# XiaokunSun/SemanticHuman

Measured on AMD Instinct MI355X. Metric: training meshes/sec at 6890 verts, batch=64, higher is better.
Workload: dtype f32

## Files before the change

include/sh_kernels.h:

```cpp
#ifndef SH_KERNELS_H
#define SH_KERNELS_H

#include <stddef.h>
#include <stdint.h>

#ifdef __cplusplus
extern "C" {
#endif

typedef void* sh_stream_t;

#if defined(__GNUC__)
#define SH_API __attribute__((visibility("default")))
#else
#define SH_API
#endif

enum sh_status {
    SH_OK = 0,
    SH_ERR_INVALID_ARG = -1,
    SH_ERR_UNSUPPORTED = -2,
    SH_ERR_WORKSPACE = -3,
    SH_ERR_LAUNCH = -4
};
// ... 142 lines not shown
SH_API int sh_grouped_linear_bwd_wgt(int G, const float* dy, int64_t y_rs, const int64_t* y_off, const float* x,
                              int64_t x_rs, const int64_t* x_off, float* const* dW, float* const* dbias, int M,
                              const int* N, const int* K, sh_stream_t stream);

SH_API size_t sh_reduce_workspace(void);

SH_API int sh_l1_loss_fwd(const float* a, const float* b, int64_t n, float* loss, void* workspace, sh_stream_t stream);
SH_API int sh_l1_loss_bwd(const float* a, const float* b, int64_t n, const float* gscale, float* grad_b, sh_stream_t stream);

SH_API int sh_vertex_l2(const float* a, const float* b, int B, int N1, int N, float scale, float* out,
                 void* workspace, sh_stream_t stream);

SH_API int sh_edge_ratio_loss_fwd(const float* x_hat, const float* x, const int32_t* faces, int B, int N1, int F,
                           float* loss, void* workspace, sh_stream_t stream);
SH_API int sh_edge_ratio_loss_bwd(const float* x_hat, const float* x, const int32_t* faces,
                           const int32_t* vptr, const int32_t* vcorner, int B, int N1, int F,
                           const float* gscale, float* grad, sh_stream_t stream);

SH_API size_t sh_recon_loss_workspace(void);
SH_API int sh_recon_loss_fwd(const float* x_hat, const float* x, const int32_t* faces, int B, int N1, int F, float edge_w,
                      float* total, float* parts, void* workspace, sh_stream_t stream);
SH_API int sh_recon_loss_bwd(const float* x_hat, const float* x, const int32_t* vptr, const int32_t* vnbr, int B, int N1, int F,
                      float edge_w, const float* gscale, float* grad, sh_stream_t stream);

SH_API int sh_part_pairdist_tile_rows(void);
SH_API int sh_part_pairdist_loss_fwd(const float* x_rec, const float* x_gt, const float* bone, const float* scale,
                              const int32_t* part_ptr, const int32_t* part_vert, const int32_t* tile_ptr,
                              const int32_t* flags, const float* w_part, int B, int N1, int P, int T, int max_part,
                              int w_mode, float w_threshold, int relat, float* loss, float* part_sum, float* part_cnt,
                              void* workspace, size_t workspace_bytes, sh_stream_t stream);
SH_API int sh_part_pairdist_loss_bwd(const float* x_rec, const float* x_gt, const float* bone, const float* scale,
                              const int32_t* part_ptr, const int32_t* part_vert, const int32_t* tile_ptr,
                              const int32_t* flags, const float* w_part, int B, int N1, int P, int T, int max_part,
                              int w_mode, float w_threshold, int relat, const float* part_cnt, const float* gscale,
                              float* grad, sh_stream_t stream);
SH_API int sh_part_pairdist_loss_fwd_grad(const float* x_rec, const float* x_gt, const float* bone, const float* scale,
                                   const int32_t* part_ptr, const int32_t* part_vert, const int32_t* tile_ptr, const int32_t* flags,
                                   const float* w_part, int B, int N1, int P, int T, int max_part, int w_mode, float w_threshold,
                                   int relat, float* loss, float* part_sum, float* part_cnt, float* grad_raw, void* workspace,
                                   size_t workspace_bytes, sh_stream_t stream);
SH_API int sh_part_pairdist_loss_bwd_scale(const float* grad_raw, const int32_t* part_ptr, const int32_t* part_vert,
                                   const float* w_part, const float* part_cnt, const float* gscale, int B, int N1, int P,
                                   int n_part_verts, float* grad, sh_stream_t stream);

SH_API int sh_measure_girth(const float* v, int64_t v_sb, const int32_t* ring_ptr, const int32_t* ring_a,
                     const int32_t* ring_b, const float* ring_f, int B, int P, float* girth, sh_stream_t stream);
// ... 186 lines not shown
SH_API int sh_spiral_conv_p3_grp(const void* xp, const int32_t* g_rows, const uint32_t* g_pos, const int32_t* g_out, int n_groups, int g_L,
                                 const void* wfrag3, const float* bias, float* y, int64_t y_sv, int64_t y_sb, void* yp, const float* yprev,
                                 int64_t yp_sv, int64_t yp_sb, const void* yprev_planes, int act, int zero_row, int backward, int B, int R,
                                 int S, int Cg, int Nout, sh_stream_t stream);

SH_API int sh_spiral_conv_bf16_rag_ok(int B, int S, int Cg, int Nout, int rag_L);
SH_API int sh_spiral_conv_bwd_data_bf16_rag(const void* dpre, int64_t dp_sv, int64_t dp_sb, const int32_t* rag_rows, const int32_t* rag_pos,
                                            int rag_L, const void* wfrag_t, void* dx, int64_t dx_sv, int64_t dx_sb, const void* yprev,
                                            int64_t yp_sv, int64_t yp_sb, int act_prev, int zero_row, int B, int n_in, int S, int Cin,
                                            int Cout, sh_stream_t stream);

SH_API int sh_spiral_conv_bwd_wgt_p3_ok(int B, int R, int S, int Cin, int Cout);
SH_API size_t sh_spiral_conv_bwd_wgt_p3_workspace(int B, int R, int S, int Cin, int Cout);
SH_API int sh_spiral_conv_bwd_wgt_p3(const void* dpre_planes, int dpre_zero_row, const void* x_planes, const int32_t* table, void* workspace,
                                     size_t workspace_bytes, int B, int R, int S, int Cin, int Cout, sh_stream_t stream);
SH_API int sh_spiral_conv_bwd_wgt_p3_presum(const void* dpre_planes, int dpre_zero_row, const void* x_planes, const int32_t* table,
                                            void* workspace, size_t workspace_bytes, const float* dpre, int64_t dp_sv, int64_t dp_sb,
                                            const int32_t* sum_rowptr, const int32_t* sum_col, const float* sum_val, float* sum_out,
                                            void* sum_out_planes, int sum_rows, int B, int R, int S, int Cin, int Cout,
                                            sh_stream_t stream);
SH_API int sh_spiral_conv_bwd_wgt_reduce_multi_kinds(int n_layers, const void* const* workspaces, float* const* dW, float* const* dbias,
                                                     const int* B, const int* R, const int* S, const int* Cin, const int* Cout,
                                                     const int* kinds, sh_stream_t stream);

#ifdef __cplusplus
}
#endif
#endif
```

semantichuman_amd/_lib.py:

```python
from __future__ import annotations

import ctypes
import os
from ctypes import c_char_p, c_float, c_int, c_int64, c_size_t, c_void_p

_HERE = os.path.dirname(os.path.abspath(__file__))
LIB_PATH = os.environ.get("SH_KERNEL_LIB") or os.path.join(_HERE, "lib", "libsh_kernels.so")

ACT_IDS = {"identity": 0, "relu": 1, "elu": 2, "leaky_relu": 3, "sigmoid": 4, "tanh": 5}

_P, _I, _L = c_void_p, c_int, c_int64
SIGNATURES = {
    "sh_version": (c_int, []),
    "sh_last_error": (c_char_p, []),
    "sh_build_id": (c_char_p, []),
    "sh_clock_probe": (c_int, [_P, _I, _I, _P]),
    "sh_profile_enable": (c_int, [_I]),
    "sh_profile_count": (c_int, []),
    "sh_profile_get": (c_int, [_I, c_char_p, _I, ctypes.POINTER(c_float)]),
    "sh_spiral_conv_fwd": (c_int, [_P, _L, _L, _P, _P, _P, _P, _L, _L, _I, _I, _I, _I, _I, _I, _I, _I, _P]),
    "sh_spiral_conv_bwd_data": (c_int, [_P, _L, _L, _P, _P, _P, _L, _L, _P, _L, _L, _I, _I, _I, _I, _I, _I, _I, _I, _P]),
    "sh_spiral_conv_bwd_data_z": (c_int, [_P, _L, _L, _I, _P, _P, _P, _L, _L, _P, _L, _L, _I, _I, _I, _I, _I, _I, _I, _I, _P]),
    "sh_weight_transpose": (c_int, [_P, _P, _I, _I, _I, _P]),
    "sh_spiral_conv_bwd_wgt_workspace": (c_size_t, [_I, _I, _I, _I, _I]),
# ... 8 lines not shown
    "sh_stack_forward": (c_int, [_I, _P, _P, _I, _I, _I, _I, _P, _P, _P, _I, _I, _P, _P, _I, _P]),
    "sh_stack_backward": (c_int, [_I, _P, _P, _I, _I, _I, _I, _P, _P, _I, _P, _P, _P, _P, _P, _P, _P, _P, _I, _I, _P, _P, _P, _P, _I, _P]),
    "sh_linear_workspace": (c_size_t, [_I, _I, _I]),
    "sh_linear_fwd": (c_int, [_P, _P, _P, _P, _I, _I, _I, _P, c_size_t, _I, _P]),
    "sh_linear_bwd_data": (c_int, [_P, _P, _P, _I, _I, _I, _P, c_size_t, _I, _P]),
    "sh_linear_bwd_wgt": (c_int, [_P, _P, _P, _P, _I, _I, _I, _P, c_size_t, _I, _P]),
    "sh_linear_bwd_wgt_adam_ok": (c_int, [_I, _I, _I]),
    "sh_linear_bwd_wgt_adam": (c_int, [_P, _I, _P, _I] + [_P] * 6 + [ctypes.c_double] * 4 + [_P, _I, _I, _I, _I, _P]),
    "sh_adam_bump": (c_int, [_I, _P, _P]),
    "sh_grouped_linear_fwd": (c_int, [_I, _P, _L, _P, _P, _P, _P, _L, _P, _I, _P, _P, _P]),
    "sh_grouped_linear_bwd_data": (c_int, [_I, _P, _L, _P, _P, _P, _L, _P, _I, _P, _P, _P]),
    "sh_grouped_linear_bwd_wgt": (c_int, [_I, _P, _L, _P, _P, _L, _P, _P, _P, _I, _P, _P, _P]),
    "sh_reduce_workspace": (c_size_t, []),
    "sh_l1_loss_fwd": (c_int, [_P, _P, _L, _P, _P, _P]),
    "sh_l1_loss_bwd": (c_int, [_P, _P, _L, _P, _P, _P]),
    "sh_vertex_l2": (c_int, [_P, _P, _I, _I, _I, c_float, _P, _P, _P]),
    "sh_edge_ratio_loss_fwd": (c_int, [_P, _P, _P, _I, _I, _I, _P, _P, _P]),
    "sh_edge_ratio_loss_bwd": (c_int, [_P, _P, _P, _P, _P, _I, _I, _I, _P, _P, _P]),
    "sh_spiral_conv_bwd_wgt_thin_ok": (c_int, [_I, _I, _I, _I, _I, _I]),
    "sh_spiral_conv_bwd_wgt_thin": (c_int, [_P, _L, _L, _P, _I, _L, _L, _P, _P, c_size_t, _P, _P, _L, _L, _P, _I, _I, _I, _I, _I, _I, _I, _I, _I, _P]),
    "sh_recon_loss_workspace": (c_size_t, []),
    "sh_recon_loss_fwd": (c_int, [_P, _P, _P, _I, _I, _I, c_float, _P, _P, _P, _P]),
    "sh_recon_loss_bwd": (c_int, [_P, _P, _P, _P, _I, _I, _I, c_float, _P, _P, _P]),
    "sh_part_pairdist_tile_rows": (c_int, []),
    "sh_part_pairdist_loss_fwd": (c_int, [_P] * 9 + [_I] * 6 + [c_float, _I, _P, _P, _P, _P, c_size_t, _P]),
    "sh_part_pairdist_loss_bwd": (c_int, [_P] * 9 + [_I] * 6 + [c_float, _I, _P, _P, _P, _P]),
    "sh_part_pairdist_loss_fwd_grad": (c_int, [_P] * 9 + [_I] * 6 + [c_float, _I, _P, _P, _P, _P, _P, c_size_t, _P]),
    "sh_part_pairdist_loss_bwd_scale": (c_int, [_P] * 6 + [_I] * 4 + [_P, _P]),
    "sh_measure_girth": (c_int, [_P, _L, _P, _P, _P, _P, _I, _I, _P, _P]),
    "sh_bone_length": (c_int, [_P, _P, _I, _I, _I, _P, _P]),
    "sh_measure_girth_bwd": (c_int, [_P, _L, _P, _P, _P, _P, _P, _P, _P, _P, _I, _P, _I, _I, _I, _P, _P]),
    "sh_bone_length_bwd": (c_int, [_P, _P, _P, _P, _P, _I, _P, _I, _I, _I, _P, _P]),
    "sh_joint_regress_bwd": (c_int, [_P, _P, _I, _I, _I, _I, _P, _P]),
    "sh_nearest_points_chunks": (c_int, [_I, _I, _I]),
    "sh_nearest_points_workspace": (c_size_t, [_I, _I, _I, _I]),
    "sh_nearest_points": (c_int, [_P, _L, _I, _P, _P, _L, _I, _P, _P, _L, _I, _I, _P, _P, _P, c_size_t, _P]),
    "sh_chamfer_fwd": (c_int, [_P, _I, _P, _P, _I, _I, _P, _L, c_float, c_float, _I, _P, _P, _P]),
    "sh_chamfer_bwd": (c_int, [_P, _L, _I, _I, _P, _L, _I, _P, _P, _P, _P, _P, _P, _L, _P, c_float, c_float, _P, _I, _P, _P]),
    "sh_nearest_surface_chunks": (c_int, [_I, _I, _I]),
    "sh_nearest_surface_workspace": (c_size_t, [_I, _I, _I, _I]),
    "sh_nearest_surface": (c_int, [_P, _L, _I, _P, _P, _L, _I, _P, _I, _P, _L, _P, _I, _I, _I, _P, _P, _P, _P, _P, c_size_t, _P]),
    "sh_chamfer_surface_bwd": (c_int, [_P, _L, _I, _I, _P, _L, _I, _P, _P, _I, _P, _P, _P, _P, _P, _P, _L, _P, c_float, c_float, _P, _I, _P, _P]),
    "sh_vertex_normals": (c_int, [_P, _L, _I, _P, _I, _P, _P, _I, _P, _P]),
    "sh_nearest_points_gated": (c_int, [_P, _L, _I, _P, _P, _L, _P, _L, _I, _P, _P, _L, _P, _L, c_float, _I, _I, _P, _P, _P, c_size_t, _P]),
    "sh_align_ranges": (c_int, [_I, _I, c_float]),
    "sh_align_partials_bytes": (c_size_t, [_I, _I, _I, c_float]),
# ... 34 lines not shown
    "sh_conv_wfrag3_bytes": (c_size_t, [_I, _I, _I]),
    "sh_conv_wfrag3_prep_multi": (c_int, [_I, _P, _P, _P, _P, _P, _P, _P]),
    "sh_spiral_conv_p3_ok": (c_int, [_I, _I, _I, _I]),
    "sh_spiral_conv_p3_kind": (c_int, [_I, _I, _I, _I]),
    "sh_p3_launch_count": (c_int64, []),
    "sh_spiral_conv_fwd_img": (c_int, [_P, _L, _L, _P, _P, _P, _P, _L, _L, _P, _I, _I, _I, _I, _I, _I, _I, _I, _P]),
    "sh_act_backward_tr_img": (c_int, [_P, _L, _L, _P, _L, _L, _P, _L, _L, _P, _I, _I, _I, _I, _I, _I, _P, _P, _P, _P, _P, _P]),
    "sh_spmm_p3": (c_int, [_P, _P, _P, _P, _L, _L, _P, _L, _L, _P, _P, _L, _L, _I, _I, _I, _I, _I, _P]),
    "sh_spiral_conv_fwd_p3": (c_int, [_P, _P, _P, _P, _P, _L, _L, _P, _I, _I, _I, _I, _I, _I, _I, _P]),
    "sh_spiral_conv_bwd_data_p3": (c_int, [_P, _I, _P, _L, _L, _I, _P, _P, _P, _L, _L, _P, _P, _L, _L, _P, _I, _I, _I, _I, _I, _I, _I, _P]),
    "sh_spiral_conv_p3_rag_ok": (c_int, [_I, _I, _I, _I, _I]),
    "sh_spiral_conv_bf16_rag_ok": (c_int, [_I, _I, _I, _I, _I]),
    "sh_spiral_conv_p3_grp_ok": (c_int, [_I, _I, _I, _I, _I]),
    "sh_spiral_conv_p3_grp_members": (c_int, [_I, _I, _I, _I]),
    "sh_spiral_conv_p3_grp_pays": (c_int, [_I, _I]),
    "sh_spiral_conv_p3_grp": (c_int, [_P, _P, _P, _P, _I, _I, _P, _P, _P, _L, _L, _P, _P, _L, _L, _P, _I, _I, _I, _I, _I, _I, _I, _I, _P]),
    "sh_spiral_conv_bwd_data_bf16_rag": (c_int, [_P, _L, _L, _P, _P, _I, _P, _P, _L, _L, _P, _L, _L, _I, _I, _I, _I, _I, _I, _I, _P]),
    "sh_spiral_conv_bwd_data_p3_rag": (c_int, [_P, _P, _P, _I, _P, _P, _L, _L, _P, _P, _L, _L, _P, _I, _I, _I, _I, _I, _I, _I, _P]),
    "sh_spiral_conv_bwd_wgt_p3_ok": (c_int, [_I, _I, _I, _I, _I]),
    "sh_spiral_conv_bwd_wgt_p3_workspace": (c_size_t, [_I, _I, _I, _I, _I]),
    "sh_spiral_conv_bwd_wgt_p3": (c_int, [_P, _I, _P, _P, _P, c_size_t, _I, _I, _I, _I, _I, _P]),
    "sh_spiral_conv_bwd_wgt_p3_presum": (c_int, [_P, _I, _P, _P, _P, c_size_t, _P, _L, _L, _P, _P, _P, _P, _P, _I, _I, _I, _I, _I, _I, _P]),
    "sh_spiral_conv_bwd_wgt_reduce_multi_kinds": (c_int, [_I, _P, _P, _P, _P, _P, _P, _P, _P, _P, _P]),
}
DTYPE_IDS = {"float32": 0, "bfloat16": 1}
FORM = {name: 1 << k for k, name in enumerate(["fwd_p3", "fwd_grp", "fwd_img", "fwd_img_only", "bwd_gimg", "bwd_thin", "bwd_p3", "bwd_rag",
                                                "bwd_grp", "bwd_ride", "bwd_presum_img", "bwd_p3w", "bwd_yimg", "bwd_in_img_only",
                                                "bwd_grad_img_only"])}



class CsrRef(ctypes.Structure):
    _fields_ = [("rowptr", c_void_p), ("col", c_void_p), ("val", c_void_p)]


class StackStep(ctypes.Structure):
    _fields_ = [("kind", c_int), ("param", c_int), ("table", c_void_p), ("table_t", c_void_p),
                ("R", c_int), ("S", c_int), ("n_in", c_int), ("cin", c_int), ("cout", c_int), ("act", c_int), ("zero_row", c_int),
                ("n1", c_int), ("n2", c_int), ("sum1", CsrRef), ("sum2", CsrRef), ("m", CsrRef), ("mt", CsrRef),
                ("m_rows", c_int), ("m_cols", c_int), ("extend", c_int),
                ("rag_rows", c_void_p), ("rag_pos", c_void_p), ("rag_L", c_int),
                ("fg_rows", c_void_p), ("fg_pos", c_void_p), ("fg_out", c_void_p), ("fg_n", c_int), ("fg_L", c_int),
                ("bg_rows", c_void_p), ("bg_pos", c_void_p), ("bg_out", c_void_p), ("bg_n", c_int), ("bg_L", c_int)]


_lib = None
# ... 100 lines not shown
```

semantichuman_amd/csrc/spiral_conv.hip:

```cpp
#include "sh_bf16.h"

#include <type_traits>

int sh_wgrad_bf16_nsplit(int B, int R, int S, int Cin, int Cout);
int sh_wgrad_p3_nslab(int B, int R, int S, int Cin, int Cout);

namespace {

constexpr int TM = 128;
constexpr int KC = 32;
constexpr int NTHREADS = 256;

struct GGParams {
    const float* x; long x_sv, x_sb;
    const int* table;
    const float* w;
    const float* bias;
    float* y; long y_sv, y_sb;
    const float* yprev; long yp_sv, yp_sb;
    int B, R, S, Cg, Nout, K;
    int Kw;
    int act;
    int zero_row;
    int log2TB, n_btiles, n_vtiles, nchunks;
// ... 1107 lines not shown
        for (; r + 48 < nslab; r += 64) {
            const float a = slab[(long)r * stride + i], b = slab[(long)(r + 16) * stride + i];
            const float c = slab[(long)(r + 32) * stride + i], d = slab[(long)(r + 48) * stride + i];
            s += (a + b) + (c + d);
        }
        for (; r < nslab; r += 16) s += slab[(long)r * stride + i];
    }
    red[ry][ox] = s;
    __syncthreads();
    if (ry == 0 && i < n) {
        float t = 0.f;
#pragma unroll
        for (int k = 0; k < 16; ++k) t += red[k][ox];
        out[i] = t;
    }
}

constexpr int MR_MAX = 32;
struct MultiReduce {
    const float* slab[MR_MAX]; long stride[MR_MAX]; long n[MR_MAX]; float* out[MR_MAX];
    int nslab[MR_MAX]; int block0[MR_MAX]; int nd;
    unsigned vec_mask;
};
__global__ __launch_bounds__(1024) void slab_reduce_multi_kernel(const MultiReduce m) {
    __shared__ f32x4 red[16][64];
    int d = 0;
    while (d + 1 < m.nd && m.block0[d + 1] <= (int)blockIdx.x) ++d;
    const float* __restrict__ slab = m.slab[d];
    const long stride = m.stride[d], n = m.n[d];
    const int nslab = m.nslab[d];
    const int ox = threadIdx.x & 63, ry = threadIdx.x >> 6;
    if ((m.vec_mask >> d) & 1u) {
        const long i = ((long)(blockIdx.x - m.block0[d]) * 64 + ox) * 4;
        f32x4 s = {0.f, 0.f, 0.f, 0.f};
        if (i < n) {
            int r = ry;
            for (; r + 48 < nslab; r += 64) {
                const f32x4 a = *reinterpret_cast<const f32x4*>(slab + (long)r * stride + i), b = *reinterpret_cast<const f32x4*>(slab + (long)(r + 16) * stride + i);
                const f32x4 c = *reinterpret_cast<const f32x4*>(slab + (long)(r + 32) * stride + i), e = *reinterpret_cast<const f32x4*>(slab + (long)(r + 48) * stride + i);
                s += (a + b) + (c + e);
            }
            for (; r < nslab; r += 16) s += *reinterpret_cast<const f32x4*>(slab + (long)r * stride + i);
        }
        red[ry][ox] = s;
        __syncthreads();
        if (ry == 0 && i < n) {
            f32x4 t = {0.f, 0.f, 0.f, 0.f};
// ... 3 lines not shown
        }
        return;
    }
    const long i = (long)(blockIdx.x - m.block0[d]) * 64 + ox;
    float s = 0.f;
    if (i < n) {
        int r = ry;
        for (; r + 48 < nslab; r += 64) {
            const float a = slab[(long)r * stride + i], b = slab[(long)(r + 16) * stride + i];
            const float c = slab[(long)(r + 32) * stride + i], e = slab[(long)(r + 48) * stride + i];
            s += (a + b) + (c + e);
        }
        for (; r < nslab; r += 16) s += slab[(long)r * stride + i];
    }
    red[ry][ox][0] = s;
    __syncthreads();
    if (ry == 0 && i < n) {
        float t = 0.f;
#pragma unroll
        for (int k = 0; k < 16; ++k) t += red[k][ox][0];
        m.out[d][i] = t;
    }
}

struct MultiTranspose {
    const float* w[MR_MAX]; float* wt[MR_MAX]; int S[MR_MAX]; int Cin[MR_MAX]; int Cout[MR_MAX]; int block0[MR_MAX]; int nd;
};
__device__ __forceinline__ void weight_transpose_block(const MultiTranspose& m, int blk) {
    int d = 0;
    while (d + 1 < m.nd && m.block0[d + 1] <= blk) ++d;
    const int S = m.S[d], Cin = m.Cin[d], Cout = m.Cout[d];
    const long n = (long)S * Cin * Cout;
    const long i = (long)(blk - m.block0[d]) * 256 + threadIdx.x;
    if (i >= n) return;
    const int co = (int)(i % Cout);
    const long t = i / Cout;
    const int s = (int)(t % S);
    const int ci = (int)(t / S);
    m.wt[d][i] = m.w[d][(long)co * S * Cin + (long)s * Cin + ci];
}
__global__ __launch_bounds__(256) void weight_transpose_multi_kernel(const MultiTranspose m) { weight_transpose_block(m, (int)blockIdx.x); }

struct WSParams {
    const float* dpre; long dp_sv, dp_sb;
    const float* x; long x_sv, x_sb;
    const int* table;
// ... 781 lines not shown
                   "sh_spiral_conv_bwd_wgt: more than 128 output channels (%d) need input channels that are a multiple of 4 (or 3)", Cout);
#define SH_WG_CASE(C, T) rc = launch_wg<C, T>(p, w, vec4, st)
    if (w.ctw == 1) {
        if (w.cot == 1) SH_WG_CASE(1, 1); else if (w.cot == 2) SH_WG_CASE(2, 1); else if (w.cot == 4) SH_WG_CASE(4, 1); else SH_WG_CASE(8, 1);
    } else {
        if (w.cot == 1) SH_WG_CASE(1, 2); else if (w.cot == 2) SH_WG_CASE(2, 2); else if (w.cot == 4) SH_WG_CASE(4, 2); else SH_WG_CASE(8, 2);
    }
    }
#undef SH_WG_CASE
    if (rc != SH_OK) return rc;
    if (!dW) return SH_OK;
    const long n = p.slab_stride;
    ShProfScope ps(st, "slab_reduce_kernel");
    SH_LAUNCH_PS(ps, slab_reduce_kernel, dim3((unsigned)((n + 63) / 64)), dim3(1024), 0, st, p.slab, p.slab_stride, w.nrc, n, dW);
    if (dbias)
        hipLaunchKernelGGL(slab_reduce_kernel, dim3((unsigned)((Cout + 63) / 64)), dim3(1024), 0, st, p.slab + p.bias_off,
                           (long)Cout, w.nrc, (long)Cout, dbias);
    SH_CHECK_LAUNCH("slab_reduce");
    return SH_OK;
}

static int reduce_multi_impl(int n_layers, const void* const* workspaces, float* const* dW, float* const* dbias, const int* B,
                             const int* R, const int* S, const int* Cin, const int* Cout, bool bf16_plan_all, sh_stream_t stream,
                             const int* kinds = nullptr) {
    SH_REQUIRE(n_layers > 0 && 2 * n_layers <= MR_MAX && workspaces && dW && dbias && B && R && S && Cin && Cout,
               SH_ERR_INVALID_ARG, "sh_spiral_conv_bwd_wgt_reduce_multi: bad argument (at most %d layers)", MR_MAX / 2);
    MultiReduce m{};
    int nd = 0, blocks = 0;
    for (int i = 0; i < n_layers; ++i) {
        SH_REQUIRE(workspaces[i] && dW[i], SH_ERR_INVALID_ARG, "sh_spiral_conv_bwd_wgt_reduce_multi: null pointer in layer %d", i);
        const int kind = kinds ? kinds[i] : (bf16_plan_all ? 1 : 0);
        SH_REQUIRE(kind >= 0 && kind <= 2, SH_ERR_INVALID_ARG, "sh_spiral_conv_bwd_wgt_reduce_multi: unknown plan kind %d of layer %d", kind, i);
        const bool bf16_plan = kind == 1;
        const int nrc = kind == 1 ? sh_wgrad_bf16_nsplit(B[i], R[i], S[i], Cin[i], Cout[i])
                        : kind == 2 ? sh_wgrad_p3_nslab(B[i], R[i], S[i], Cin[i], Cout[i]) : plan_wgrad(B[i], R[i], S[i], Cin[i], Cout[i]).nrc;
        SH_REQUIRE(nrc > 0, SH_ERR_UNSUPPORTED, "sh_spiral_conv_bwd_wgt_reduce_multi: layer %d has no plan of kind %d", i, kind);
        const long stride = (long)Cout[i] * S[i] * Cin[i];
        const float* slab = static_cast<const float*>(workspaces[i]);
        m.slab[nd] = slab; m.stride[nd] = stride; m.nslab[nd] = nrc; m.n[nd] = stride; m.out[nd] = dW[i]; m.block0[nd] = blocks;
        static const int vec_on = sh_env_int("SH_SLAB_REDUCE_VEC", 1, 0, 2);
        if ((vec_on == 2 || (vec_on == 1 && (nrc >= 512 || bf16_plan))) && stride % 4 == 0 && ((reinterpret_cast<uintptr_t>(slab) | reinterpret_cast<uintptr_t>(dW[i])) & 15) == 0) {
            m.vec_mask |= 1u << nd;
            blocks += (int)((stride / 4 + 63) / 64);
        } else
            blocks += (int)((stride + 63) / 64);
        ++nd;
        if (dbias[i]) {
            m.slab[nd] = slab + (long)nrc * stride; m.stride[nd] = Cout[i]; m.nslab[nd] = nrc; m.n[nd] = Cout[i];
            m.out[nd] = dbias[i]; m.block0[nd] = blocks;
            blocks += (Cout[i] + 63) / 64; ++nd;
        }
    }
    m.nd = nd;
    hipStream_t st = static_cast<hipStream_t>(stream);
    ShProfScope ps(st, "slab_reduce_multi_kernel");
    SH_LAUNCH_PS(ps, slab_reduce_multi_kernel, dim3((unsigned)blocks), dim3(1024), 0, st, m);
    SH_CHECK_LAUNCH("slab_reduce_multi");
    return SH_OK;
}

int sh_spiral_conv_bwd_wgt_reduce_multi(int n_layers, const void* const* workspaces, float* const* dW, float* const* dbias,
                                        const int* B, const int* R, const int* S, const int* Cin, const int* Cout,
                                        sh_stream_t stream) {
    return reduce_multi_impl(n_layers, workspaces, dW, dbias, B, R, S, Cin, Cout, false, stream);
}

int sh_spiral_conv_bwd_wgt_reduce_multi_kinds(int n_layers, const void* const* workspaces, float* const* dW, float* const* dbias,
                                              const int* B, const int* R, const int* S, const int* Cin, const int* Cout,
                                              const int* kinds, sh_stream_t stream) {
    SH_REQUIRE(kinds, SH_ERR_INVALID_ARG, "sh_spiral_conv_bwd_wgt_reduce_multi_kinds: no kinds");
    return reduce_multi_impl(n_layers, workspaces, dW, dbias, B, R, S, Cin, Cout, false, stream, kinds);
}

int sh_spiral_conv_bwd_wgt_reduce_multi_bf16(int n_layers, const void* const* workspaces, float* const* dW, float* const* dbias,
                                             const int* B, const int* R, const int* S, const int* Cin, const int* Cout,
                                             sh_stream_t stream) {
    return reduce_multi_impl(n_layers, workspaces, dW, dbias, B, R, S, Cin, Cout, true, stream);
}

int sh_weight_transpose_multi(int n_layers, const float* const* weight, float* const* weight_t, const int* S, const int* Cin,
                              const int* Cout, sh_stream_t stream) {
    SH_REQUIRE(n_layers > 0 && n_layers <= MR_MAX && weight && weight_t && S && Cin && Cout, SH_ERR_INVALID_ARG,
               "sh_weight_transpose_multi: bad argument (at most %d layers)", MR_MAX);
    MultiTranspose m{};
    int blocks = 0;
    for (int i = 0; i < n_layers; ++i) {
        SH_REQUIRE(weight[i] && weight_t[i] && S[i] > 0 && Cin[i] > 0 && Cout[i] > 0, SH_ERR_INVALID_ARG,
                   "sh_weight_transpose_multi: bad layer %d", i);
        m.w[i] = weight[i]; m.wt[i] = weight_t[i]; m.S[i] = S[i]; m.Cin[i] = Cin[i]; m.Cout[i] = Cout[i]; m.block0[i] = blocks;
        blocks += (int)(((long)S[i] * Cin[i] * Cout[i] + 255) / 256);
    }
    m.nd = n_layers;
    hipLaunchKernelGGL(weight_transpose_multi_kernel, dim3((unsigned)blocks), dim3(256), 0, static_cast<hipStream_t>(stream), m);
    SH_CHECK_LAUNCH("weight_transpose_multi");
// ... 65 lines not shown
```

semantichuman_amd/csrc/spmm_loss.hip:

```cpp
#include "sh_bf16.h"

namespace {

constexpr int RED_BLOCKS = 2048;

template <bool VEC, bool P3 = false>
__global__ __launch_bounds__(256) void spmm_kernel(const int* __restrict__ rowptr, const int* __restrict__ col,
                                                   const float* __restrict__ val, const float* __restrict__ x, long x_sv, long x_sb,
                                                   float* __restrict__ y, long y_sv, long y_sb, const float* __restrict__ yprev,
                                                   long yp_sv, long yp_sb, int act, int zero_row, int B, int rows, int C,
                                                   char* __restrict__ img = nullptr, long img_vb = 0, long img_bgb = 0) {
    const int CW = VEC ? C >> 2 : C;
    const int per_row = B * CW;
    const int parts = (per_row + 255) >> 8;
    const long items = (long)rows * parts;
    for (long it = blockIdx.x; it < items; it += gridDim.x) {
        const int r = (int)(it / parts), part = (int)(it - (long)r * parts);
        const int e0 = rowptr[r], e1 = rowptr[r + 1];
        const bool zero = r == zero_row;
        for (int j = part * 256 + threadIdx.x; j < per_row && j < (part + 1) * 256; j += 256) {
            const int b = j / CW, cw = j - b * CW;
            const int co = VEC ? 4 * cw : cw;
            const long xo = (long)b * x_sb + co;
            const long yo = (long)r * y_sv + (long)b * y_sb + co;
// ... 219 lines not shown
}

__global__ void edge_loss_bwd_kernel(const float* __restrict__ xh, const float* __restrict__ x, const int* __restrict__ faces,
                                     const int* __restrict__ vptr, const int* __restrict__ vcorner, int B, int N1, int F,
                                     const float* __restrict__ gscale, float* __restrict__ grad) {
    const float sc = gscale[0] / ((float)B * (float)F);
    const long n = (long)B * N1;
    for (long i = (long)blockIdx.x * blockDim.x + threadIdx.x; i < n; i += (long)gridDim.x * blockDim.x) {
        const long bb = i / N1;
        const int v = (int)(i - bb * N1);
        const float* ph = xh + bb * N1 * 3;
        const float* pg = x + bb * N1 * 3;
        float g[3] = {0.f, 0.f, 0.f};
        for (int e = vptr[v]; e < vptr[v + 1]; ++e) {
            const int c = vcorner[e], f = c / 3, kx = c - 3 * f;
            const int o1 = faces[3 * f + (kx + 1) % 3], o2 = faces[3 * f + (kx + 2) % 3];
            edge_grad(ph, pg, v, o1, g);
            edge_grad(ph, pg, v, o2, g);
        }
        grad[i * 3] = sc * g[0]; grad[i * 3 + 1] = sc * g[1]; grad[i * 3 + 2] = sc * g[2];
    }
}

__global__ void recon_partial_kernel(const float* __restrict__ xh, const float* __restrict__ x, const int* __restrict__ faces,
                                     int B, int N1, int F, float* __restrict__ part) {
    __shared__ float red[16];
    float s = 0.f;
    const long n = (long)B * N1 * 3;
    for (long i = (long)blockIdx.x * blockDim.x + threadIdx.x; i < n; i += (long)gridDim.x * blockDim.x) s += fabsf(x[i] - xh[i]);
    const float t1 = block_sum(s, red);
    if (threadIdx.x == 0) part[blockIdx.x] = t1;
    __syncthreads();
    s = 0.f;
    const long nf = (long)B * F;
    for (long i = (long)blockIdx.x * blockDim.x + threadIdx.x; i < nf; i += (long)gridDim.x * blockDim.x) {
        const long bb = i / F;
        const int f = (int)(i - bb * F);
        const I3 fc = *reinterpret_cast<const I3*>(faces + 3 * f);
        const float* ph = xh + bb * N1 * 3;
        const float* pg = x + bb * N1 * 3;
        const P3 ha = ld3(ph, fc.a), hb = ld3(ph, fc.b), hc = ld3(ph, fc.c), ga = ld3(pg, fc.a), gb = ld3(pg, fc.b), gc = ld3(pg, fc.c);
        s += fabsf(edge_len3(ha, hb) / (edge_len3(ga, gb) + 0.00001f) - 1.f);
        s += fabsf(edge_len3(hb, hc) / (edge_len3(gb, gc) + 0.00001f) - 1.f);
        s += fabsf(edge_len3(ha, hc) / (edge_len3(ga, gc) + 0.00001f) - 1.f);
    }
    const float t2 = block_sum(s, red);
    if (threadIdx.x == 0) part[RED_BLOCKS + blockIdx.x] = t2;
}

__global__ void recon_final_kernel(const float* __restrict__ part, int np, double scale1, double scale2, float w, float* __restrict__ total,
                                   float* __restrict__ parts) {
    __shared__ double red[2][256];
    double s1 = 0.0, s2 = 0.0;
    for (int i = threadIdx.x; i < np; i += 256) { s1 += (double)part[i]; s2 += (double)part[RED_BLOCKS + i]; }
    red[0][threadIdx.x] = s1; red[1][threadIdx.x] = s2;
    __syncthreads();
    for (int o = 128; o > 0; o >>= 1) {
        if ((int)threadIdx.x < o) { red[0][threadIdx.x] += red[0][threadIdx.x + o]; red[1][threadIdx.x] += red[1][threadIdx.x + o]; }
        __syncthreads();
    }
    if (threadIdx.x == 0) {
        const float rec = (float)(red[0][0] * scale1), edge = (float)(red[1][0] * scale2);
        total[0] = rec + w * edge; parts[0] = rec; parts[1] = edge;
    }
}

__global__ __launch_bounds__(256) void recon_bwd_kernel(const float* __restrict__ xh, const float* __restrict__ x, const int* __restrict__ vptr,
                                                        const int* __restrict__ vnbr, int B, int N1, int F, float w,
                                                        const float* __restrict__ gscale, float* __restrict__ grad) {
    const float g0 = gscale[0];
    const float s1 = g0 / ((float)B * (float)N1 * 3.f), s2 = g0 * w / ((float)B * (float)F);
    const long n = (long)B * N1;
    for (long i = (long)blockIdx.x * blockDim.x + threadIdx.x; i < n; i += (long)gridDim.x * blockDim.x) {
        const long bb = i / N1;
        const int v = (int)(i - bb * N1);
        const float* ph = xh + bb * N1 * 3;
        const float* pg = x + bb * N1 * 3;
        const int p0 = 2 * vptr[v], p1 = 2 * vptr[v + 1];
        const P3 hv = ld3(ph, v), gv = ld3(pg, v);
        float g[3] = {0.f, 0.f, 0.f};
        for (int e = p0; e < p1; e += 4) {
            int o[4];
            P3 ho[4], go[4];
#pragma unroll
            for (int k = 0; k < 4; ++k) o[k] = vnbr[e + k < p1 ? e + k : p1 - 1];
#pragma unroll
            for (int k = 0; k < 4; ++k) { ho[k] = ld3(ph, o[k]); go[k] = ld3(pg, o[k]); }
#pragma unroll
            for (int k = 0; k < 4; ++k)
                if (e + k < p1) edge_grad3(hv, gv, ho[k], go[k], g);
        }
        const float df[3] = {hv.x - gv.x, hv.y - gv.y, hv.z - gv.z};
        P3 o3;
        o3.x = s2 * g[0] + (df[0] > 0.f ? s1 : (df[0] < 0.f ? -s1 : 0.f));
        o3.y = s2 * g[1] + (df[1] > 0.f ? s1 : (df[1] < 0.f ? -s1 : 0.f));
        o3.z = s2 * g[2] + (df[2] > 0.f ? s1 : (df[2] < 0.f ? -s1 : 0.f));
        *reinterpret_cast<P3*>(grad + i * 3) = o3;
    }
}

inline int grid_for(long n, int per_block) {
    long g = (n + per_block - 1) / per_block;
    if (g < 1) g = 1;
    return (int)(g < 2048 ? g : 2048);
}

}

extern "C" {

int sh_spmm(const int32_t* rowptr, const int32_t* col, const float* val, const float* x, int64_t x_sv, int64_t x_sb, float* y,
            int64_t y_sv, int64_t y_sb, const float* yprev, int64_t yp_sv, int64_t yp_sb, int act_prev, int zero_row, int B,
            int rows, int C, sh_stream_t stream) {
// ... 74 lines not shown
    const int nb = grid_for(n, 1024) < RED_BLOCKS ? grid_for(n, 1024) : RED_BLOCKS;
    hipLaunchKernelGGL(vertex_l2_partial_kernel, dim3(nb), dim3(256), 0, st, a, b, B, N1, N, scale, part);
    hipLaunchKernelGGL(final_sum_kernel, dim3(1), dim3(256), 0, st, part, nb, 1.0 / (double)n, out);
    SH_CHECK_LAUNCH("vertex_l2");
    return SH_OK;
}

int sh_edge_ratio_loss_fwd(const float* x_hat, const float* x, const int32_t* faces, int B, int N1, int F, float* loss,
                           void* workspace, sh_stream_t stream) {
    SH_REQUIRE(x_hat && x && faces && loss && workspace && B > 0 && N1 > 0 && F > 0, SH_ERR_INVALID_ARG,
               "sh_edge_ratio_loss_fwd: bad argument");
    hipStream_t st = static_cast<hipStream_t>(stream);
    float* part = static_cast<float*>(workspace);
    const long n = (long)B * F;
    const int nb = grid_for(n, 1024) < RED_BLOCKS ? grid_for(n, 1024) : RED_BLOCKS;
    hipLaunchKernelGGL(edge_loss_partial_kernel, dim3(nb), dim3(256), 0, st, x_hat, x, faces, B, N1, F, part);
    hipLaunchKernelGGL(final_sum_kernel, dim3(1), dim3(256), 0, st, part, nb, 1.0 / (double)n, loss);
    SH_CHECK_LAUNCH("edge_ratio_loss_fwd");
    return SH_OK;
}

size_t sh_recon_loss_workspace(void) { return (size_t)2 * RED_BLOCKS * sizeof(float); }

int sh_recon_loss_fwd(const float* x_hat, const float* x, const int32_t* faces, int B, int N1, int F, float edge_w, float* total,
                      float* parts, void* workspace, sh_stream_t stream) {
    SH_REQUIRE(x_hat && x && faces && total && parts && workspace && B > 0 && N1 > 0 && F > 0, SH_ERR_INVALID_ARG,
               "sh_recon_loss_fwd: bad argument");
    hipStream_t st = static_cast<hipStream_t>(stream);
    float* part = static_cast<float*>(workspace);
    const long n = (long)B * N1 * 3;
    const int nb = grid_for(n, 1024) < RED_BLOCKS ? grid_for(n, 1024) : RED_BLOCKS;
    hipLaunchKernelGGL(recon_partial_kernel, dim3(nb), dim3(256), 0, st, x_hat, x, faces, B, N1, F, part);
    hipLaunchKernelGGL(recon_final_kernel, dim3(1), dim3(256), 0, st, part, nb, 1.0 / (double)n, 1.0 / ((double)B * F), edge_w, total, parts);
    SH_CHECK_LAUNCH("recon_loss_fwd");
    return SH_OK;
}

int sh_recon_loss_bwd(const float* x_hat, const float* x, const int32_t* vptr, const int32_t* vnbr, int B, int N1, int F, float edge_w,
                      const float* gscale, float* grad, sh_stream_t stream) {
    SH_REQUIRE(x_hat && x && vptr && vnbr && gscale && grad && B > 0 && N1 > 0 && F > 0, SH_ERR_INVALID_ARG,
               "sh_recon_loss_bwd: bad argument");
    const long n = (long)B * N1;
    hipLaunchKernelGGL(recon_bwd_kernel, dim3(grid_for(n, 256)), dim3(256), 0, static_cast<hipStream_t>(stream), x_hat, x, vptr, vnbr, B,
                       N1, F, edge_w, gscale, grad);
    SH_CHECK_LAUNCH("recon_loss_bwd");
    return SH_OK;
}

int sh_edge_ratio_loss_bwd(const float* x_hat, const float* x, const int32_t* faces, const int32_t* vptr, const int32_t* vcorner,
                           int B, int N1, int F, const float* gscale, float* grad, sh_stream_t stream) {
    SH_REQUIRE(x_hat && x && faces && vptr && vcorner && gscale && grad && B > 0 && N1 > 0 && F > 0, SH_ERR_INVALID_ARG,
               "sh_edge_ratio_loss_bwd: bad argument");
    const long n = (long)B * N1;
    hipLaunchKernelGGL(edge_loss_bwd_kernel, dim3(grid_for(n, 256)), dim3(256), 0, static_cast<hipStream_t>(stream), x_hat, x, faces,
                       vptr, vcorner, B, N1, F, gscale, grad);
    SH_CHECK_LAUNCH("edge_ratio_loss_bwd");
    return SH_OK;
}

}
```

Before: 47950.

## Rework recon loss and slab reduce kernels with XCD-contiguous blocks and deeper prefetch

Three paths change. The recon loss forward now prefetches face indices ahead of use and unrolls the elementwise loop, and the backward batches 16 neighbour indices and issues 8 gathers at a time. Both remap block IDs so consecutive blocks land on the same XCD, aiming to improve L2 locality and hide gather latency. The multi-layer slab reduction moves from 1024-thread to 256-thread workgroups with wider per-thread loads, and vectorises the bias slabs. The old kernels stay reachable through environment variables and form arguments, at the cost of higher register pressure from the deeper unrolling.

```diff
diff --git a/include/sh_kernels.h b/include/sh_kernels.h
--- a/include/sh_kernels.h
+++ b/include/sh_kernels.h
@@ -188,6 +188,10 @@
                       float* total, float* parts, void* workspace, sh_stream_t stream);
 SH_API int sh_recon_loss_bwd(const float* x_hat, const float* x, const int32_t* vptr, const int32_t* vnbr, int B, int N1, int F,
                       float edge_w, const float* gscale, float* grad, sh_stream_t stream);
+SH_API int sh_recon_loss_fwd_form(const float* x_hat, const float* x, const int32_t* faces, int B, int N1, int F, float edge_w,
+                           float* total, float* parts, void* workspace, int form, sh_stream_t stream);
+SH_API int sh_recon_loss_bwd_form(const float* x_hat, const float* x, const int32_t* vptr, const int32_t* vnbr, int B, int N1, int F,
+                           float edge_w, const float* gscale, float* grad, int form, sh_stream_t stream);
 
 SH_API int sh_part_pairdist_tile_rows(void);
 SH_API int sh_part_pairdist_loss_fwd(const float* x_rec, const float* x_gt, const float* bone, const float* scale,
@@ -420,6 +424,9 @@
 SH_API int sh_spiral_conv_bwd_wgt_reduce_multi_kinds(int n_layers, const void* const* workspaces, float* const* dW, float* const* dbias,
                                                      const int* B, const int* R, const int* S, const int* Cin, const int* Cout,
                                                      const int* kinds, sh_stream_t stream);
+SH_API int sh_spiral_conv_bwd_wgt_reduce_multi_form(int n_layers, const void* const* workspaces, float* const* dW, float* const* dbias,
+                                                    const int* B, const int* R, const int* S, const int* Cin, const int* Cout,
+                                                    const int* kinds, int form, sh_stream_t stream);
 
 #ifdef __cplusplus
 }
diff --git a/semantichuman_amd/_lib.py b/semantichuman_amd/_lib.py
--- a/semantichuman_amd/_lib.py
+++ b/semantichuman_amd/_lib.py
@@ -54,6 +54,8 @@
     "sh_recon_loss_workspace": (c_size_t, []),
     "sh_recon_loss_fwd": (c_int, [_P, _P, _P, _I, _I, _I, c_float, _P, _P, _P, _P]),
     "sh_recon_loss_bwd": (c_int, [_P, _P, _P, _P, _I, _I, _I, c_float, _P, _P, _P]),
+    "sh_recon_loss_fwd_form": (c_int, [_P, _P, _P, _I, _I, _I, c_float, _P, _P, _P, _I, _P]),
+    "sh_recon_loss_bwd_form": (c_int, [_P, _P, _P, _P, _I, _I, _I, c_float, _P, _P, _I, _P]),
     "sh_part_pairdist_tile_rows": (c_int, []),
     "sh_part_pairdist_loss_fwd": (c_int, [_P] * 9 + [_I] * 6 + [c_float, _I, _P, _P, _P, _P, c_size_t, _P]),
     "sh_part_pairdist_loss_bwd": (c_int, [_P] * 9 + [_I] * 6 + [c_float, _I, _P, _P, _P, _P]),
@@ -134,6 +136,7 @@
     "sh_spiral_conv_bwd_wgt_p3": (c_int, [_P, _I, _P, _P, _P, c_size_t, _I, _I, _I, _I, _I, _P]),
     "sh_spiral_conv_bwd_wgt_p3_presum": (c_int, [_P, _I, _P, _P, _P, c_size_t, _P, _L, _L, _P, _P, _P, _P, _P, _I, _I, _I, _I, _I, _I, _P]),
     "sh_spiral_conv_bwd_wgt_reduce_multi_kinds": (c_int, [_I, _P, _P, _P, _P, _P, _P, _P, _P, _P, _P]),
+    "sh_spiral_conv_bwd_wgt_reduce_multi_form": (c_int, [_I, _P, _P, _P, _P, _P, _P, _P, _P, _P, _I, _P]),
 }
 DTYPE_IDS = {"float32": 0, "bfloat16": 1}
 FORM = {name: 1 << k for k, name in enumerate(["fwd_p3", "fwd_grp", "fwd_img", "fwd_img_only", "bwd_gimg", "bwd_thin", "bwd_p3", "bwd_rag",
diff --git a/semantichuman_amd/csrc/spiral_conv.hip b/semantichuman_amd/csrc/spiral_conv.hip
--- a/semantichuman_amd/csrc/spiral_conv.hip
+++ b/semantichuman_amd/csrc/spiral_conv.hip
@@ -1153,7 +1153,7 @@
     int nslab[MR_MAX]; int block0[MR_MAX]; int nd;
     unsigned vec_mask;
 };
-__global__ __launch_bounds__(1024) void slab_reduce_multi_kernel(const MultiReduce m) {
+__global__ __launch_bounds__(1024) void slab_reduce_multi_wg1024_kernel(const MultiReduce m) {
     __shared__ f32x4 red[16][64];
     int d = 0;
     while (d + 1 < m.nd && m.block0[d + 1] <= (int)blockIdx.x) ++d;
@@ -1203,6 +1203,62 @@
         m.out[d][i] = t;
     }
 }
+
+template <typename T, int LX, int KW>
+__device__ __forceinline__ void slab_reduce_wg256(const float* __restrict__ slab, long stride, long n, int nslab, long blk,
+                                                  float* __restrict__ out, T* red) {
+    constexpr int V = (int)(sizeof(T) / sizeof(float)), PPT = LX / 16;
+    const int ox = threadIdx.x % LX, ty = threadIdx.x / LX;
+    const long i = (blk * LX + ox) * V;
+    T s[PPT];
+#pragma unroll
+    for (int j = 0; j < PPT; ++j) s[j] = T{};
+    if (i < n) {
+        const float* p = slab + i;
+        for (int r0 = ty * PPT; r0 < nslab; r0 += 16 * KW) {
+            T v[PPT][KW];
+#pragma unroll
+            for (int j = 0; j < PPT; ++j)
+#pragma unroll
+                for (int k = 0; k < KW; ++k) {
+                    const int r = r0 + j + 16 * k;
+                    v[j][k] = T{};
+                    if (r < nslab) v[j][k] = *reinterpret_cast<const T*>(p + (long)r * stride);
+                }
+#pragma unroll
+            for (int j = 0; j < PPT; ++j)
+#pragma unroll
+                for (int g = 0; g < KW / 4; ++g) {
+                    const int r = r0 + j + 64 * g;
+                    if (r + 48 < nslab) s[j] += (v[j][4 * g] + v[j][4 * g + 1]) + (v[j][4 * g + 2] + v[j][4 * g + 3]);
+                    else {
+#pragma unroll
+                        for (int q = 0; q < 3; ++q)
+                            if (r + 16 * q < nslab) s[j] += v[j][4 * g + q];
+                    }
+                }
+        }
+    }
+#pragma unroll
+    for (int j = 0; j < PPT; ++j) red[(ty * PPT + j) * LX + ox] = s[j];
+    __syncthreads();
+    if (ty == 0 && i < n) {
+        T t = T{};
+#pragma unroll
+        for (int k = 0; k < 16; ++k) t += red[k * LX + ox];
+        *reinterpret_cast<T*>(out + i) = t;
+    }
+}
+template <int KW>
+__device__ __forceinline__ void slab_reduce_multi_body(const MultiReduce& m) {
+    __shared__ f32x4 red[256];
+    int d = 0;
+    while (d + 1 < m.nd && m.block0[d + 1] <= (int)blockIdx.x) ++d;
+    const long blk = (long)(blockIdx.x - m.block0[d]);
+    if ((m.vec_mask >> d) & 1u) slab_reduce_wg256<f32x4, 16, KW>(m.slab[d], m.stride[d], m.n[d], m.nslab[d], blk, m.out[d], red);
+    else slab_reduce_wg256<float, 64, 4>(m.slab[d], m.stride[d], m.n[d], m.nslab[d], blk, m.out[d], reinterpret_cast<float*>(red));
+}
+__global__ __launch_bounds__(256) void slab_reduce_multi_kernel(const MultiReduce m) { slab_reduce_multi_body<16>(m); }
 
 struct MultiTranspose {
     const float* w[MR_MAX]; float* wt[MR_MAX]; int S[MR_MAX]; int Cin[MR_MAX]; int Cout[MR_MAX]; int block0[MR_MAX]; int nd;
@@ -2030,11 +2086,12 @@
 
 static int reduce_multi_impl(int n_layers, const void* const* workspaces, float* const* dW, float* const* dbias, const int* B,
                              const int* R, const int* S, const int* Cin, const int* Cout, bool bf16_plan_all, sh_stream_t stream,
-                             const int* kinds = nullptr) {
+                             const int* kinds = nullptr, int form = -1) {
     SH_REQUIRE(n_layers > 0 && 2 * n_layers <= MR_MAX && workspaces && dW && dbias && B && R && S && Cin && Cout,
                SH_ERR_INVALID_ARG, "sh_spiral_conv_bwd_wgt_reduce_multi: bad argument (at most %d layers)", MR_MAX / 2);
     MultiReduce m{};
     int nd = 0, blocks = 0;
+    bool wg1024 = false;
     for (int i = 0; i < n_layers; ++i) {
         SH_REQUIRE(workspaces[i] && dW[i], SH_ERR_INVALID_ARG, "sh_spiral_conv_bwd_wgt_reduce_multi: null pointer in layer %d", i);
         const int kind = kinds ? kinds[i] : (bf16_plan_all ? 1 : 0);
@@ -2047,7 +2104,12 @@
         const float* slab = static_cast<const float*>(workspaces[i]);
         m.slab[nd] = slab; m.stride[nd] = stride; m.nslab[nd] = nrc; m.n[nd] = stride; m.out[nd] = dW[i]; m.block0[nd] = blocks;
         static const int vec_on = sh_env_int("SH_SLAB_REDUCE_VEC", 1, 0, 2);
-        if ((vec_on == 2 || (vec_on == 1 && (nrc >= 512 || bf16_plan))) && stride % 4 == 0 && ((reinterpret_cast<uintptr_t>(slab) | reinterpret_cast<uintptr_t>(dW[i])) & 15) == 0) {
+        static const int form_env = sh_env_int("SH_SLAB_REDUCE_FORM", 0, 0, 1);
+        wg1024 = (form < 0 ? form_env : form) == 1;
+        if (!wg1024) {
+            if (stride % 4 == 0 && ((reinterpret_cast<uintptr_t>(slab) | reinterpret_cast<uintptr_t>(dW[i])) & 15) == 0) m.vec_mask |= 1u << nd;
+            blocks += (int)((stride + 63) / 64);
+        } else if ((vec_on == 2 || (vec_on == 1 && (nrc >= 512 || bf16_plan))) && stride % 4 == 0 && ((reinterpret_cast<uintptr_t>(slab) | reinterpret_cast<uintptr_t>(dW[i])) & 15) == 0) {
             m.vec_mask |= 1u << nd;
             blocks += (int)((stride / 4 + 63) / 64);
         } else
@@ -2056,13 +2118,16 @@
         if (dbias[i]) {
             m.slab[nd] = slab + (long)nrc * stride; m.stride[nd] = Cout[i]; m.nslab[nd] = nrc; m.n[nd] = Cout[i];
             m.out[nd] = dbias[i]; m.block0[nd] = blocks;
+            if (!wg1024 && Cout[i] % 4 == 0 && ((reinterpret_cast<uintptr_t>(m.slab[nd]) | reinterpret_cast<uintptr_t>(dbias[i])) & 15) == 0)
+                m.vec_mask |= 1u << nd;
             blocks += (Cout[i] + 63) / 64; ++nd;
         }
     }
     m.nd = nd;
     hipStream_t st = static_cast<hipStream_t>(stream);
     ShProfScope ps(st, "slab_reduce_multi_kernel");
-    SH_LAUNCH_PS(ps, slab_reduce_multi_kernel, dim3((unsigned)blocks), dim3(1024), 0, st, m);
+    if (wg1024) SH_LAUNCH_PS(ps, slab_reduce_multi_wg1024_kernel, dim3((unsigned)blocks), dim3(1024), 0, st, m);
+    else SH_LAUNCH_PS(ps, slab_reduce_multi_kernel, dim3((unsigned)blocks), dim3(256), 0, st, m);
     SH_CHECK_LAUNCH("slab_reduce_multi");
     return SH_OK;
 }
@@ -2078,6 +2143,13 @@
                                               const int* kinds, sh_stream_t stream) {
     SH_REQUIRE(kinds, SH_ERR_INVALID_ARG, "sh_spiral_conv_bwd_wgt_reduce_multi_kinds: no kinds");
     return reduce_multi_impl(n_layers, workspaces, dW, dbias, B, R, S, Cin, Cout, false, stream, kinds);
+}
+
+int sh_spiral_conv_bwd_wgt_reduce_multi_form(int n_layers, const void* const* workspaces, float* const* dW, float* const* dbias,
+                                             const int* B, const int* R, const int* S, const int* Cin, const int* Cout,
+                                             const int* kinds, int form, sh_stream_t stream) {
+    SH_REQUIRE(form == 0 || form == 1, SH_ERR_INVALID_ARG, "sh_spiral_conv_bwd_wgt_reduce_multi_form: unknown form %d", form);
+    return reduce_multi_impl(n_layers, workspaces, dW, dbias, B, R, S, Cin, Cout, false, stream, kinds, form);
 }
 
 int sh_spiral_conv_bwd_wgt_reduce_multi_bf16(int n_layers, const void* const* workspaces, float* const* dW, float* const* dbias,
diff --git a/semantichuman_amd/csrc/spmm_loss.hip b/semantichuman_amd/csrc/spmm_loss.hip
--- a/semantichuman_amd/csrc/spmm_loss.hip
+++ b/semantichuman_amd/csrc/spmm_loss.hip
@@ -265,7 +265,7 @@
     }
 }
 
-__global__ void recon_partial_kernel(const float* __restrict__ xh, const float* __restrict__ x, const int* __restrict__ faces,
+__global__ void recon_partial_serial_kernel(const float* __restrict__ xh, const float* __restrict__ x, const int* __restrict__ faces,
                                      int B, int N1, int F, float* __restrict__ part) {
     __shared__ float red[16];
     float s = 0.f;
@@ -291,6 +291,69 @@
     if (threadIdx.x == 0) part[RED_BLOCKS + blockIdx.x] = t2;
 }
 
+__device__ __forceinline__ int xcd_contiguous_block(int p, int nb) {
+    const int x = p & 7, q = nb >> 3, rem = nb & 7;
+    return x * q + (x < rem ? x : rem) + (p >> 3);
+}
+
+template <int UF>
+__global__ __launch_bounds__(256) void recon_partial_kernel(const float* __restrict__ xh, const float* __restrict__ x, const int* __restrict__ faces,
+                                                            int B, int N1, int F, float* __restrict__ part, int xcd) {
+    __shared__ float red[16];
+    constexpr int U = 4;
+    const int blk = xcd ? xcd_contiguous_block((int)blockIdx.x, (int)gridDim.x) : (int)blockIdx.x;
+    const long G = (long)gridDim.x * 256, i0 = (long)blk * 256 + threadIdx.x;
+    const long n = (long)B * N1 * 3, nf = (long)B * F;
+    I3 fc[UF];
+    long fb[UF];
+    auto face_indices = [&](long i) {
+#pragma unroll
+        for (int k = 0; k < UF; ++k) {
+            const long j = i + k * G < nf ? i + k * G : 0;
+            const long bb = j / F;
+            fc[k] = *reinterpret_cast<const I3*>(faces + 3 * (int)(j - bb * F));
+            fb[k] = bb * N1 * 3;
+        }
+    };
+    face_indices(i0);
+    float s = 0.f;
+    for (long i = i0; i < n; i += U * G) {
+        float a[U], b[U];
+#pragma unroll
+        for (int k = 0; k < U; ++k) {
+            const long j = i + k * G < n ? i + k * G : i;
+            a[k] = x[j]; b[k] = xh[j];
+        }
+#pragma unroll
+        for (int k = 0; k < U; ++k)
+            if (i + k * G < n) s += fabsf(a[k] - b[k]);
+    }
+    const float t1 = block_sum(s, red);
+    if (threadIdx.x == 0) part[blk] = t1;
+    __syncthreads();
+    s = 0.f;
+    for (long i = i0; i < nf; i += UF * G) {
+        P3 ha[UF], hb[UF], hc[UF], ga[UF], gb[UF], gc[UF];
+#pragma unroll
+        for (int k = 0; k < UF; ++k) {
+            const float* ph = xh + fb[k];
+            const float* pg = x + fb[k];
+            ha[k] = ld3(ph, fc[k].a); hb[k] = ld3(ph, fc[k].b); hc[k] = ld3(ph, fc[k].c);
+            ga[k] = ld3(pg, fc[k].a); gb[k] = ld3(pg, fc[k].b); gc[k] = ld3(pg, fc[k].c);
+        }
+        if (i + UF * G < nf) face_indices(i + UF * G);
+#pragma unroll
+        for (int k = 0; k < UF; ++k)
+            if (i + k * G < nf) {
+                s += fabsf(edge_len3(ha[k], hb[k]) / (edge_len3(ga[k], gb[k]) + 0.00001f) - 1.f);
+                s += fabsf(edge_len3(hb[k], hc[k]) / (edge_len3(gb[k], gc[k]) + 0.00001f) - 1.f);
+                s += fabsf(edge_len3(ha[k], hc[k]) / (edge_len3(ga[k], gc[k]) + 0.00001f) - 1.f);
+            }
+    }
+    const float t2 = block_sum(s, red);
+    if (threadIdx.x == 0) part[RED_BLOCKS + blk] = t2;
+}
+
 __global__ void recon_final_kernel(const float* __restrict__ part, int np, double scale1, double scale2, float w, float* __restrict__ total,
                                    float* __restrict__ parts) {
     __shared__ double red[2][256];
@@ -308,7 +371,7 @@
     }
 }
 
-__global__ __launch_bounds__(256) void recon_bwd_kernel(const float* __restrict__ xh, const float* __restrict__ x, const int* __restrict__ vptr,
+__global__ __launch_bounds__(256) void recon_bwd_depth4_kernel(const float* __restrict__ xh, const float* __restrict__ x, const int* __restrict__ vptr,
                                                         const int* __restrict__ vnbr, int B, int N1, int F, float w,
                                                         const float* __restrict__ gscale, float* __restrict__ grad) {
     const float g0 = gscale[0];
@@ -332,6 +395,46 @@
 #pragma unroll
             for (int k = 0; k < 4; ++k)
                 if (e + k < p1) edge_grad3(hv, gv, ho[k], go[k], g);
+        }
+        const float df[3] = {hv.x - gv.x, hv.y - gv.y, hv.z - gv.z};
+        P3 o3;
+        o3.x = s2 * g[0] + (df[0] > 0.f ? s1 : (df[0] < 0.f ? -s1 : 0.f));
+        o3.y = s2 * g[1] + (df[1] > 0.f ? s1 : (df[1] < 0.f ? -s1 : 0.f));
+        o3.z = s2 * g[2] + (df[2] > 0.f ? s1 : (df[2] < 0.f ? -s1 : 0.f));
+        *reinterpret_cast<P3*>(grad + i * 3) = o3;
+    }
+}
+
+template <int W, int D>
+__global__ __launch_bounds__(256) void recon_bwd_kernel(const float* __restrict__ xh, const float* __restrict__ x, const int* __restrict__ vptr,
+                                                        const int* __restrict__ vnbr, int B, int N1, int F, float w,
+                                                        const float* __restrict__ gscale, float* __restrict__ grad, int xcd) {
+    const float g0 = gscale[0];
+    const float s1 = g0 / ((float)B * (float)N1 * 3.f), s2 = g0 * w / ((float)B * (float)F);
+    const long n = (long)B * N1;
+    const int blk = xcd ? xcd_contiguous_block((int)blockIdx.x, (int)gridDim.x) : (int)blockIdx.x;
+    for (long i = (long)blk * 256 + threadIdx.x; i < n; i += (long)gridDim.x * 256) {
+        const long bb = i / N1;
+        const int v = (int)(i - bb * N1);
+        const float* ph = xh + bb * N1 * 3;
+        const float* pg = x + bb * N1 * 3;
+        const int p0 = 2 * vptr[v], p1 = 2 * vptr[v + 1];
+        const P3 hv = ld3(ph, v), gv = ld3(pg, v);
+        float g[3] = {0.f, 0.f, 0.f};
+        for (int e = p0; e < p1; e += W) {
+            int o[W];
+#pragma unroll
+            for (int k = 0; k < W; ++k) o[k] = vnbr[e + k < p1 ? e + k : p1 - 1];
+#pragma unroll
+            for (int h = 0; h < W; h += D) {
+                if (e + h >= p1) break;
+                P3 ho[D], go[D];
+#pragma unroll
+                for (int k = 0; k < D; ++k) { ho[k] = ld3(ph, o[h + k]); go[k] = ld3(pg, o[h + k]); }
+#pragma unroll
+                for (int k = 0; k < D; ++k)
+                    if (e + h + k < p1) edge_grad3(hv, gv, ho[k], go[k], g);
+            }
         }
         const float df[3] = {hv.x - gv.x, hv.y - gv.y, hv.z - gv.z};
         P3 o3;
@@ -452,15 +555,28 @@
 
 size_t sh_recon_loss_workspace(void) { return (size_t)2 * RED_BLOCKS * sizeof(float); }
 
+static int recon_form(int form) {
+    static const int form_env = sh_env_int("SH_RECON_FORM", 0, 0, 2);
+    return form < 0 ? form_env : form;
+}
+
 int sh_recon_loss_fwd(const float* x_hat, const float* x, const int32_t* faces, int B, int N1, int F, float edge_w, float* total,
                       float* parts, void* workspace, sh_stream_t stream) {
+    return sh_recon_loss_fwd_form(x_hat, x, faces, B, N1, F, edge_w, total, parts, workspace, -1, stream);
+}
+
+int sh_recon_loss_fwd_form(const float* x_hat, const float* x, const int32_t* faces, int B, int N1, int F, float edge_w, float* total,
+                           float* parts, void* workspace, int form, sh_stream_t stream) {
+    SH_REQUIRE(form >= -1 && form <= 2, SH_ERR_INVALID_ARG, "sh_recon_loss_fwd_form: unknown form %d", form);
+    form = recon_form(form);
     SH_REQUIRE(x_hat && x && faces && total && parts && workspace && B > 0 && N1 > 0 && F > 0, SH_ERR_INVALID_ARG,
                "sh_recon_loss_fwd: bad argument");
     hipStream_t st = static_cast<hipStream_t>(stream);
     float* part = static_cast<float*>(workspace);
     const long n = (long)B * N1 * 3;
     const int nb = grid_for(n, 1024) < RED_BLOCKS ? grid_for(n, 1024) : RED_BLOCKS;
-    hipLaunchKernelGGL(recon_partial_kernel, dim3(nb), dim3(256), 0, st, x_hat, x, faces, B, N1, F, part);
+    if (form == 1) hipLaunchKernelGGL(recon_partial_serial_kernel, dim3(nb), dim3(256), 0, st, x_hat, x, faces, B, N1, F, part);
+    else hipLaunchKernelGGL(recon_partial_kernel<2>, dim3(nb), dim3(256), 0, st, x_hat, x, faces, B, N1, F, part, form != 2 ? 1 : 0);
     hipLaunchKernelGGL(recon_final_kernel, dim3(1), dim3(256), 0, st, part, nb, 1.0 / (double)n, 1.0 / ((double)B * F), edge_w, total, parts);
     SH_CHECK_LAUNCH("recon_loss_fwd");
     return SH_OK;
@@ -468,11 +584,20 @@
 
 int sh_recon_loss_bwd(const float* x_hat, const float* x, const int32_t* vptr, const int32_t* vnbr, int B, int N1, int F, float edge_w,
                       const float* gscale, float* grad, sh_stream_t stream) {
+    return sh_recon_loss_bwd_form(x_hat, x, vptr, vnbr, B, N1, F, edge_w, gscale, grad, -1, stream);
+}
+
+int sh_recon_loss_bwd_form(const float* x_hat, const float* x, const int32_t* vptr, const int32_t* vnbr, int B, int N1, int F, float edge_w,
+                           const float* gscale, float* grad, int form, sh_stream_t stream) {
+    SH_REQUIRE(form >= -1 && form <= 2, SH_ERR_INVALID_ARG, "sh_recon_loss_bwd_form: unknown form %d", form);
+    form = recon_form(form);
     SH_REQUIRE(x_hat && x && vptr && vnbr && gscale && grad && B > 0 && N1 > 0 && F > 0, SH_ERR_INVALID_ARG,
                "sh_recon_loss_bwd: bad argument");
     const long n = (long)B * N1;
-    hipLaunchKernelGGL(recon_bwd_kernel, dim3(grid_for(n, 256)), dim3(256), 0, static_cast<hipStream_t>(stream), x_hat, x, vptr, vnbr, B,
-                       N1, F, edge_w, gscale, grad);
+    hipStream_t st = static_cast<hipStream_t>(stream);
+    if (form == 1) hipLaunchKernelGGL(recon_bwd_depth4_kernel, dim3(grid_for(n, 256)), dim3(256), 0, st, x_hat, x, vptr, vnbr, B, N1, F, edge_w, gscale, grad);
+#define SH_BWD(W, D, X) hipLaunchKernelGGL((recon_bwd_kernel<W, D>), dim3(grid_for(n, 256)), dim3(256), 0, st, x_hat, x, vptr, vnbr, B, N1, F, edge_w, gscale, grad, X)
+    else SH_BWD(16, 8, form != 2 ? 1 : 0);
     SH_CHECK_LAUNCH("recon_loss_bwd");
     return SH_OK;
 }
```

New measurement: 48210 (median of 6 runs). Within noise of the previous version (+0.6%).
